# SuwoongHeo/neurecon

Measured on AMD Instinct MI355X. Metric: rays/sec (4096 rays x 128 samples, 8-layer x256 SDF MLP), higher is better.
Workload: dtype f16x3

## Files before the change

### neurecon_amd/csrc/nr_mlp.hip

```cpp
#include <algorithm>
#include <type_traits>
#include "nr_common.h"
#include "nr_mlp.h"
#include "nr_tgemm.h"

namespace nr {

using lds_ptr = __attribute__((address_space(3))) void*;

__device__ __forceinline__ void glds16(const char* gsrc, uint32_t lds_addr) {
  unsigned keep;
  asm volatile(
      "s_mov_b32 %0, m0\n\t"
      "s_mov_b32 m0, %2\n\t"
      "s_nop 0\n\t"
      "global_load_lds_dwordx4 %1, off\n\t"
      "s_mov_b32 m0, %0"
      : "=&s"(keep)
      : "v"(gsrc), "s"(lds_addr)
      : "memory");
}

__device__ __forceinline__ void glds16s(const char* sbase, uint32_t voff, uint32_t lds_addr) {
  unsigned keep;
// ... 398 lines not shown
    if (main) {
      if (e_cur) {
        const float4* eb = ws.slab_cur();
        const float4 e0 = eb[lane], e1 = eb[64 + lane];
        y0 = make_float4(act_bwd<P, ACTB>(y0.x, e0.x), act_bwd<P, ACTB>(y0.y, e0.y), act_bwd<P, ACTB>(y0.z, e0.z),
                         act_bwd<P, ACTB>(y0.w, e0.w));
        y1 = make_float4(act_bwd<P, ACTB>(y1.x, e1.x), act_bwd<P, ACTB>(y1.y, e1.y), act_bwd<P, ACTB>(y1.z, e1.z),
                         act_bwd<P, ACTB>(y1.w, e1.w));
      }
      if constexpr (NBO1 > 0) push2<NBO1>(Y, y0, y1);
    } else {
      emb(2 * c - NBO1, y0);
      emb(2 * c + 1 - NBO1, y1);
    }
    ws.flip();
  }
}

__device__ __noinline__ float embed_feature(int f, float x0, float x1, float x2, int nfreq) {
  if (f < 3) return f == 0 ? x0 : (f == 1 ? x1 : x2);
  const int fp = f - 3;
  if (fp >= 6 * nfreq) return 0.0f;
  const int band = fp / 6, m = fp - band * 6, c = m % 3;
  const float xc = c == 0 ? x0 : (c == 1 ? x1 : x2);
  const float v = fmul(xc, (float)(1 << band));
  return m < 3 ? sinf(v) : cosf(v);
}
__device__ __noinline__ void embed_backward(int f, float gf, float x0, float x1, float x2, int nfreq, float& n0,
                                            float& n1, float& n2) {
  float contrib;
  int c;
  if (f < 3) {
    contrib = gf;
    c = f;
  } else {
    const int fp = f - 3;
    if (fp >= 6 * nfreq) return;
    const int band = fp / 6, m = fp - band * 6;
    c = m % 3;
    const float freq = (float)(1 << band);
    const float xc = c == 0 ? x0 : (c == 1 ? x1 : x2);
    const float v = fmul(xc, freq);
    contrib = m < 3 ? fmul(fmul(gf, cosf(v)), freq) : fmul(fmul(gf, -sinf(v)), freq);
  }
  if (c == 0) n0 = fadd(n0, contrib);
  else if (c == 1) n1 = fadd(n1, contrib);
  else n2 = fadd(n2, contrib);
}

__device__ __forceinline__ float wave_sum4(float v) {
  v += __shfl_xor(v, 16);
  v += __shfl_xor(v, 32);
  return v;
}

struct SdfKArgs {
  const char* packed;
  SdfLayout L;
  const float* pts;
  int64_t P;
  float* sdf;
  float* nabla;
  float* feature;
  float4* scratch;
  int nfreq;
  const int* P_dev;
  int P_mult;
  float4* slabs;
  const int* tiles;
  const int* n_tiles;
  const char* f8_alt;
};

template <int P, bool NABLA>
__global__ __launch_bounds__(kThreads) void sdf_kernel(SdfKArgs a) {
  constexpr int CB = chunk_bytes(18);
  __shared__ __attribute__((aligned(16))) char smem[kRing * CB + (NABLA ? 2 * kSlabChunk : 0)];
  WStream<CB> ws{smem, NABLA ? smem + kRing * CB : nullptr, 0, 0, 0};
  const int lane = threadIdx.x & 63, wave = __builtin_amdgcn_readfirstlane(threadIdx.x >> 6);
  const int j = lane & 15, g = lane >> 4;
  const SdfLayout& L = a.L;
  const char* W = a.packed;
  auto OP = [&](int i) { return W + L.op_off[i]; };
  auto OPB = [&](int i) { return (int)L.op_bytes[i]; };
  const float* w8 = (const float*)(W + L.w8row0_off);
  const float b8 = *(const float*)(W + L.misc_off);
  float4* escr = uniform_ptr(a.scratch + (size_t)(blockIdx.x * kWaves + wave) * (8 * 16 * 64));
  const bool want_feat = a.feature != nullptr;

  ws.start(OP(F0), OPB(F0), OP(F0) + OPB(F0), OPB(F0));

  const int64_t Pn = a.P_dev ? min(a.P, (int64_t)(*a.P_dev) * a.P_mult) : a.P;
  for (int64_t base = (int64_t)blockIdx.x * kPointsPerWG; base < Pn; base += (int64_t)gridDim.x * kPointsPerWG) {
    const bool has_next = base + (int64_t)gridDim.x * kPointsPerWG < Pn;
    const int64_t p = base + wave * kTile + j;
    const bool valid = p < Pn;
    const int64_t pc = valid ? p : Pn - 1;
    const float x0 = a.pts[pc * 3 + 0], x1 = a.pts[pc * 3 + 1], x2 = a.pts[pc * 3 + 2];

    float4 E[4];
#pragma unroll
    for (int b = 0; b < 4; ++b) {
      const int f = 16 * b + 4 * g;
      E[b] = make_float4(embed_feature(f + 0, x0, x1, x2, a.nfreq), embed_feature(f + 1, x0, x1, x2, a.nfreq),
                         embed_feature(f + 2, x0, x1, x2, a.nfreq), embed_feature(f + 3, x0, x1, x2, a.nfreq));
    }
// ... 376 lines not shown
      wait_vmcnt(n);
    }
    __syncthreads();
    cur = nextr(cur);
  }
  __device__ __forceinline__ void flip_nowait() {
    __syncthreads();
    cur = nextr(cur);
  }
};

__device__ __forceinline__ f16x8 rd_frag(const float4* __restrict__ A, int i, int lane) {
  return as_h8(A[i * 64 + lane]);
}
template <int NS, class Stage>
__device__ __forceinline__ void mma4(const float4* __restrict__ A, const f16x8 (&bh)[kNC][12],
                                     const f16x8 (&bl)[kNC][12], f32x4 (&acc)[kNC][2], int lane, Stage&& stage) {
  f16x8 nh0 = rd_frag(A, 0, lane), nl0 = rd_frag(A, 1, lane);
  f16x8 nh1 = rd_frag(A, NS * 2, lane), nl1 = rd_frag(A, NS * 2 + 1, lane);
#pragma unroll
  for (int s = 0; s < NS; ++s) {
    const f16x8 h0 = nh0, l0 = nl0, h1 = nh1, l1 = nl1;
    if (s + 1 < NS) {
      nh0 = rd_frag(A, (s + 1) * 2, lane);
      nl0 = rd_frag(A, (s + 1) * 2 + 1, lane);
      nh1 = rd_frag(A, (NS + s + 1) * 2, lane);
      nl1 = rd_frag(A, (NS + s + 1) * 2 + 1, lane);
    }
    stage(s);
#pragma unroll
    for (int q = 0; q < kNC; ++q) {
      acc[q][0] = mfma16h(l0, bh[q][s], acc[q][0]);
      acc[q][1] = mfma16h(l1, bh[q][s], acc[q][1]);
      acc[q][0] = mfma16h(h0, bl[q][s], acc[q][0]);
      acc[q][1] = mfma16h(h1, bl[q][s], acc[q][1]);
      acc[q][0] = mfma16h(h0, bh[q][s], acc[q][0]);
      acc[q][1] = mfma16h(h1, bh[q][s], acc[q][1]);
    }
    if (s + 1 < NS) __builtin_amdgcn_sched_group_barrier(0x100, 4, 0);
    __builtin_amdgcn_sched_group_barrier(0x008, 6 * kNC, 0);
    __builtin_amdgcn_sched_barrier(0);
  }
}

struct Z4 {
  float4 z[kNC][2];
  float4 aux[2];
};

constexpr float kT = 144.26944f;
constexpr float kC = 0.0069314749f;

#ifdef NR_EXP_STAMPS
constexpr int kStampPh = 6;
__device__ unsigned long long g_nr_stamps[2048 * 8 * kStampPh];
__device__ __forceinline__ unsigned long long* stamp_lds() {
  __shared__ unsigned long long s_stamp[kW4 * kStampPh];
  return s_stamp;
}
__device__ __forceinline__ uint64_t stamp_now() { return __builtin_amdgcn_s_memtime(); }
__device__ __forceinline__ void stamp_add(int ph, uint64_t dt) {
  if ((threadIdx.x & 63) == 0) stamp_lds()[(threadIdx.x >> 6) * kStampPh + ph] += dt;
}
#define NR_STAMP(var) const uint64_t var = stamp_now()
#else
#define NR_STAMP(var)
#endif

enum { kSlot = 0, kLean = 1, kTab = 2 };
template <int KB, int NBO, int NXT_CB, bool AUX, bool TS, int MODE = kSlot, int NXT_MODE = kSlot, class WS,
          class Pre, class Epi>
__device__ __forceinline__ void op4(WS& ws, const char* __restrict__ op, const char* nxt, const f16x8 (&bh)[kNC][12],
                                    const f16x8 (&bl)[kNC][12], const float (&xinv)[kNC], Pend4& pd, Pre&& pre,
                                    Epi&& epi, int lane, float winv = 0.0f) {
  constexpr int CB = chunk_bytes(KB);
  constexpr bool LEAN = MODE == kLean;
  constexpr int FB = MODE != kSlot ? weight_bytes(KB) : CB;
  constexpr int NXT_FB = NXT_MODE != kSlot ? NXT_CB - 1024 : NXT_CB;
  static_assert(!LEAN || (!AUX && !TS), "lean ops carry no per-row data");
  constexpr int NCH = NBO / 2;
  static_assert(MODE != kTab || NCH * 512 <= kTabBytes, "bias table entries");
  constexpr int LA = WS::kRingN - 1;
  static_assert(NCH >= 2, "the 2-ahead stream needs >= 2 chunks per op");
  const int g = lane >> 4;
  Z4 zq{};
#pragma unroll
  for (int c = 0; c < NCH; ++c) {
    const char* opc = op;
    const char* nxc = nxt;
    asm volatile("" : "+s"(opc), "+s"(nxc));
    NR_STAMP(t0);
    int npend = 0;
    if (c + LA < NCH) {
      ws.template issue<FB>(opc + (c + LA) * CB);
      npend = WS::template npieces<FB>();
    } else if (nxc) {
      ws.template issue<NXT_FB>(nxc + (c + LA - NCH) * NXT_CB);
      npend = WS::template npieces<NXT_FB>();
      if constexpr (NXT_MODE == kTab) {
        if (c + LA == NCH) {
          ws.template dma_tab<NXT_CB>(nxc, ws.tcur ^ 1);
          npend += WS::ntab();
        }
      }
    }
    npend += pre(c);
    npend += pd.flush();
    NR_STAMP(t1);
    const float4* A = ws.buf();
    f32x4 acc[kNC][2] = {};
    mma4<KB / 2>(A, bh, bl, acc, lane, [&](int st) {
      if (c > 0) {
#pragma unroll
        for (int e = 0; e < 8; ++e)
          if (e * (KB / 2) / 8 == st) epi(c - 1, zq, e);
      }
    });
    NR_STAMP(t2);
    float wi;
// ... 190 lines not shown
};

template <int NMAIN, class WS>
struct BwdEpi4 {
  f16x8 (&oh)[kNC][12];
  f16x8 (&ol)[kNC][12];
  const float (&sc)[kNC];
  WS& ws;
  float4* park;
  int park_blk;
  float (&mrun)[kNC];
  Pend4& pd;
  int lane;
  int plane;
  float4 y[kNC][2];
  __device__ __forceinline__ void operator()(int c, const Z4& zz, int st) {
    if (2 * c < NMAIN) {
      const int q = st >> 2, k = st & 3;
      if (q >= kNC) return;
      if (k < 2) {
        const uint4 sw = *(const uint4*)((const char*)ws.slab_read() + ((kNC * k + q) * 64 + lane) * 16);
        y[q][k] = unpack24_mul(sw.x, sw.y, sw.z, zz.z[q][k]);
      } else if (k == 2) {
        mrun[q] = amax8(mrun[q], y[q][0], y[q][1]);
      } else {
        split8a(y[q][0], y[q][1], sc[q], oh[q][c], ol[q][c]);
        if (q == kNC - 1) ws.slab_consumed();
      }
    } else if (st == 7) {
#pragma unroll
      for (int q = 0; q < kNC; ++q) {
        pd.v[q] = zz.z[q][0];
        pd.v[kNC + q] = zz.z[q][1];
      }
      pend_chunk(pd, park, park_blk + 2 * c - NMAIN, plane, false);
    }
  }
};

struct NoPre4 {
  __device__ __forceinline__ int operator()(int) const { return 0; }
};

template <bool NABLA, bool FEAT, int STAGE_>
__global__ __attribute__((amdgpu_flat_work_group_size(STAGE_ == 3 ? 256 : kT4, STAGE_ == 3 ? 256 : kT4),
                          amdgpu_waves_per_eu(kWPE, kWPE)))
void sdf4_kernel(SdfKArgs a) {
  constexpr int STAGE = STAGE_ == 3 ? 0 : (STAGE_ == 4 ? 2 : STAGE_);
  constexpr bool COMPACT = STAGE_ == 4;
  constexpr int NW = STAGE_ == 3 ? 4 : kW4;
  static_assert(STAGE_ != 3 || (!NABLA && !FEAT), "narrow tiles: forward-only launches");
  static_assert(STAGE == 0 || (NABLA && !FEAT), "deferred nablas: no feature");
  constexpr int PPW = 16 * kNC * NW;
  constexpr int CB = chunk_bytes(18);
  constexpr int C16 = chunk_bytes(16), C4 = chunk_bytes(4), C14 = chunk_bytes(14), C18 = chunk_bytes(18);
  static_assert((size_t)kW4 * kNC * kSlabColBytes <= kScratchPerWG, "per-workgroup slab scratch");
  constexpr bool SLABS = NABLA && STAGE != 1;
  constexpr int RING = SLABS ? 3 : kFwdRing;
  constexpr bool TABF = !SLABS;
  constexpr int FM = TABF ? kTab : kSlot;
  constexpr int LDSB = RING * CB + (SLABS ? kSlabRing * kSlab4 : 0) + (TABF ? 2 * kTabBytes : 0);
  __shared__ __attribute__((aligned(16))) char smem[LDSB];
  static_assert(LDSB <= 160 * 1024, "LDS budget");
  static_assert(!TABF || RING * CB + 2 * kTabBytes == LDSB, "the bias table follows the weight ring");
  WStream4<CB, RING, NW> ws{smem, SLABS ? smem + RING * CB : nullptr, 0, 0, 0, 0, TABF ? smem + RING * CB : nullptr, 0};
  const int lane = threadIdx.x & 63, wave = __builtin_amdgcn_readfirstlane(threadIdx.x >> 6);
  const int j = lane & 15, g = lane >> 4;
  const char* W = a.packed;
  auto OP = [&](int i) {
    const char* w = W;
    asm volatile("" : "+s"(w));
    return w + sdf_op_off(i);
  };
  auto OPF8 = [&]() {
    const char* w = a.f8_alt;
    asm volatile("" : "+s"(w));
    return w ? w : OP(F8);
  };
  const float b8 = *(const float*)(W + a.L.misc_off);
  float4* escr = uniform_ptr((float4*)((char*)a.scratch + (size_t)(blockIdx.x * kW4 + wave) * (kNC * kSlabColBytes)));
  auto slab = [&](int l) {
    char* e = (char*)escr;
    asm volatile("" : "+s"(e));
    return (float4*)(e + l * kNC * kSlab24Layer);
  };

#ifdef NR_EXP_STAMPS
  if ((threadIdx.x & 63) == 0)
    for (int i = 0; i < kStampPh; ++i) stamp_lds()[wave * kStampPh + i] = 0;
#endif
  constexpr bool LEANR = STAGE == 2 || (NABLA && FEAT);
  constexpr int W16 = weight_bytes(16);
  if constexpr (STAGE == 2) ws.template start<W16, W16>(OP(B7), OP(B7) + C16);
  else if constexpr (TABF)
    ws.template start<weight_bytes(4), weight_bytes(4), weight_bytes(4), C4>(OP(F0), OP(F0) + C4, OP(F0) + 2 * C4, OP(F0));
  else ws.template start<C4, C4>(OP(F0), OP(F0) + C4);
  Pend4 pd{};
  NoPre4 nopre;
  const float kSpSlack = 0.0070f;

  const int64_t Pn = COMPACT      ? ((int64_t)(*a.n_tiles) + 15) / 16 * 16
                     : STAGE == 2 ? (int64_t)(*a.n_tiles) * kPointsPerWG / kW4
                                  : (a.P_dev ? min(a.P, (int64_t)(*a.P_dev) * a.P_mult) : a.P);
  for (int64_t base = (int64_t)blockIdx.x * PPW; base < Pn; base += (int64_t)gridDim.x * PPW) {
    const bool has_next = base + (int64_t)gridDim.x * PPW < Pn;
    int64_t p0 = base + wave * 16 * kNC;
    int plane = lane;
    uint32_t soff = 0;
    int64_t pl = 0;
    bool listed = true;
    if constexpr (COMPACT) {
      const int64_t n = *a.n_tiles;
      const int64_t w0 = p0 < n ? p0 : n - 16;
      const int e = a.tiles[w0 + j];
      const int e0 = __builtin_amdgcn_readfirstlane(a.tiles[w0]);
      listed = p0 < n && e >= 0;
      pl = e >= 0 ? e : e0;
      const uint32_t rt = (uint32_t)((pl >> 4) - (e0 >> 4)), js = (uint32_t)(pl & 15);
      plane = (int)(rt * (uint32_t)(kSlabColBytes / 16) + js + 16u * (uint32_t)g);
      soff = rt * (uint32_t)kSlabColBytes + (js + 16u * (uint32_t)g) * (uint32_t)kSlabVB;
      escr = uniform_ptr((float4*)((char*)a.slabs + (size_t)(e0 >> 4) * kSlabColBytes));
    } else if constexpr (STAGE == 2) {
      const int64_t ti = min(p0 / 16, (int64_t)(*a.n_tiles) - 1);
      const int64_t tile = a.tiles[ti];
      escr = uniform_ptr((float4*)((char*)a.slabs + (size_t)tile * kSlabColBytes));
      p0 = p0 / 16 < (int64_t)(*a.n_tiles) ? tile * 16 : a.P;
    } else if constexpr (STAGE == 1) {
      escr = uniform_ptr((float4*)((char*)a.slabs + (size_t)(p0 / 16) * kSlabColBytes));
    }
    const int64_t Pv = STAGE == 2 ? a.P : Pn;
    int64_t pq[kNC];
    bool valid[kNC];
    float xs[kNC][3];
#pragma unroll
    for (int q = 0; q < kNC; ++q) {
      const int64_t p = p0 + 16 * q + j;
      if constexpr (COMPACT) {
        valid[q] = listed;
        pq[q] = pl;
      } else {
        valid[q] = p < Pv;
        pq[q] = valid[q] ? p : Pv - 1;
      }
      xs[q][0] = a.pts[pq[q] * 3 + 0];
      xs[q][1] = a.pts[pq[q] * 3 + 1];
      xs[q][2] = a.pts[pq[q] * 3 + 2];
    }
    float4 E[kNC][4];
    float mE[kNC], xinv[kNC];
    f16x8 Uh[kNC][12], Ul[kNC][12], Vh[kNC][12], Vl[kNC][12];
    float mrun[kNC], m_in[kNC];
    auto next_scales = [&](int kb, float extra, const float (&floor_max)[kNC], float (&sc)[kNC]) {
      const float4 v = TABF ? ws.tab_entry(0)[8] : ws.buf()[2 * kb * 64 + 8];
#pragma unroll
      for (int q = 0; q < kNC; ++q) sc[q] = bound_scale(fmaxf(fmaf(v.y, m_in[q], v.z) + extra, floor_max[q]));
    };
    struct OpScal {
      float winv, R, B;
    };
    auto op_scal = [&](int opi) {
      const char* w = W;
      asm volatile("" : "+s"(w));
      typedef __attribute__((address_space(4))) const float cfloat;
      cfloat* rb = (cfloat*)(w + a.L.bound_off + 8 * opi);
      return OpScal{*(cfloat*)(w + a.L.winv_off + 4 * opi), rb[0], rb[1]};
    };
    auto finish = [&](const float (&sc)[kNC], float mscale = 1.0f) {
#pragma unroll
      for (int q = 0; q < kNC; ++q) {
        m_in[q] = max4_groups(mrun[q]) * mscale;
        mrun[q] = 0.0f;
        xinv[q] = 1.0f / sc[q];
      }
    };
    float zero2[kNC];
#pragma unroll
    for (int q = 0; q < kNC; ++q) zero2[q] = 0.0f;
    if constexpr (STAGE != 2) {
#pragma unroll
    for (int q = 0; q < kNC; ++q) {
#pragma unroll
      for (int b = 0; b < 4; ++b) {
        const int f = 16 * b + 4 * g;
        E[q][b] = make_float4(embed_feature(f + 0, xs[q][0], xs[q][1], xs[q][2], a.nfreq),
                              embed_feature(f + 1, xs[q][0], xs[q][1], xs[q][2], a.nfreq),
                              embed_feature(f + 2, xs[q][0], xs[q][1], xs[q][2], a.nfreq),
                              embed_feature(f + 3, xs[q][0], xs[q][1], xs[q][2], a.nfreq));
      }
      mE[q] = max4_groups(amax8(amax8(0.0f, E[q][0], E[q][1]), E[q][2], E[q][3]));
      const float sE = bound_scale(mE[q]);
      split8a(E[q][0], E[q][1], sE, Uh[q][0], Ul[q][0]);
      split8a(E[q][2], E[q][3], sE, Uh[q][1], Ul[q][1]);
      xinv[q] = 1.0f / sE;
    }
    float4* epark = slab(7);
    if constexpr (NABLA) {
      const uint32_t l = opaque_lane(lane);
#pragma unroll
      for (int q = 0; q < kNC; ++q)
#pragma unroll
        for (int b = 0; b < 4; ++b) {
          const uint32_t off = (((12 + b) * kNC + q) * 64 + l) * 16u;
          const f32x4 d = tof(E[q][b]);
          asm volatile("global_store_dwordx4 %0, %1, %2\n\ts_nop 1" : : "v"(off), "v"(d), "s"(epark) : "memory");
        }
    }
#pragma unroll
    for (int q = 0; q < kNC; ++q) {
      mrun[q] = 0.0f;
      m_in[q] = mE[q];
    }
    auto fwd_epi = [&](f16x8(&oh)[kNC][12], f16x8(&ol)[kNC][12], const float (&sc)[kNC], float4* sl) {
      return FwdEpi4<NABLA>{oh, ol, sc, sl, mrun, pd, lane};
    };

    {
      float sc[kNC];
      next_scales(4, kSpSlack, zero2, sc);
      op4<4, 16, C16, false, true, FM, FM>(ws, OP(F0), OP(F1), Uh, Ul, xinv, pd, nopre, fwd_epi(Vh, Vl, sc, slab(0)), lane);
      finish(sc, kC);
    }
    {
      float sc[kNC];
      next_scales(16, kSpSlack, zero2, sc);
      op4<16, 16, C16, false, true, FM, FM>(ws, OP(F1), OP(F2), Vh, Vl, xinv, pd, nopre, fwd_epi(Uh, Ul, sc, slab(1)), lane);
      finish(sc, kC);
    }
    {
      float sc[kNC];
      next_scales(16, kSpSlack, zero2, sc);
      op4<16, 16, C16, false, true, FM, FM>(ws, OP(F2), OP(F3), Uh, Ul, xinv, pd, nopre, fwd_epi(Vh, Vl, sc, slab(2)), lane);
      finish(sc, kC);
    }
    {
      float sc[kNC];
      next_scales(16, kSpSlack, mE, sc);
      op4<16, 14, C18, false, true, FM, FM>(ws, OP(F3), OP(F4), Vh, Vl, xinv, pd, nopre, fwd_epi(Uh, Ul, sc, slab(3)), lane);
      if constexpr (NABLA) {
        asm volatile("s_waitcnt vmcnt(0)" ::: "memory");
#pragma unroll
        for (int q = 0; q < kNC; ++q)
#pragma unroll
          for (int b = 0; b < 4; ++b) E[q][b] = fromf(*((const gf4*)epark + ((12 + b) * kNC + q) * 64 + lane));
      }
#pragma unroll
      for (int q = 0; q < kNC; ++q) {
        split8a(E[q][0], E[q][1], sc[q], Uh[q][7], Ul[q][7]);
        split8a(E[q][2], E[q][3], sc[q], Uh[q][8], Ul[q][8]);
        mrun[q] = fmaxf(mrun[q], mE[q] * (1.0f / kC));
      }
      finish(sc, kC);
    }
    {
      float sc[kNC];
      next_scales(18, kSpSlack, zero2, sc);
      op4<18, 16, C16, false, true, FM, FM>(ws, OP(F4), OP(F5), Uh, Ul, xinv, pd, nopre, fwd_epi(Vh, Vl, sc, slab(4)), lane);
      finish(sc, kC);
    }
    {
      float sc[kNC];
      next_scales(16, kSpSlack, zero2, sc);
      op4<16, 16, C16, false, true, FM, FM>(ws, OP(F5), OP(F6), Vh, Vl, xinv, pd, nopre, fwd_epi(Uh, Ul, sc, slab(5)), lane);
      finish(sc, kC);
    }
    {
      float sc[kNC];
      next_scales(16, kSpSlack, zero2, sc);
      op4<16, 16, C16, false, true, FM, FM>(ws, OP(F6), OP(F7), Uh, Ul, xinv, pd, nopre, fwd_epi(Vh, Vl, sc, slab(6)), lane);
      finish(sc, kC);
    }
    float sdf_part[kNC];
#pragma unroll
    for (int q = 0; q < kNC; ++q) sdf_part[q] = 0.0f;
    {
      float sc[kNC];
      next_scales(16, kSpSlack, zero2, sc);
      F7Epi4<NABLA, FEAT> epi{Uh, Ul, sc, slab(7), mrun, sdf_part, pd, lane};
      constexpr int NXT = ((NABLA && STAGE == 0) || FEAT) ? C16 : C4;
      const char* n;
      if constexpr (FEAT) n = OPF8();
      else n = (NABLA && STAGE == 0) ? OP(B7) : (has_next ? OP(F0) : nullptr);
      op4<16, 16, NXT, true, false, FM, FM>(ws, OP(F7), n, Vh, Vl, xinv, pd, nopre, epi, lane);
      finish(sc);
    }
#pragma unroll
    for (int q = 0; q < kNC; ++q) {
      const float sdf = wave_sum4(sdf_part[q]) + b8;
      if (valid[q] && g == 0) a.sdf[p0 + 16 * q + j] = sdf;
    }
    if constexpr (FEAT) {
      const int64_t pf = p0 < Pn ? p0 : Pn - 1;
      float4* fb = uniform_ptr((float4*)(a.feature + pf * 256));
      uint32_t frow[kNC];
#pragma unroll
      for (int q = 0; q < kNC; ++q) frow[q] = (uint32_t)(pq[q] - pf);
      auto epi = [&](int c, const Z4& zz, int st) {
        if (st != 7) return;
#pragma unroll
        for (int q = 0; q < kNC; ++q) {
          pd.v[2 * q] = zz.z[q][0];
          pd.v[2 * q + 1] = zz.z[q][1];
          const uint32_t r = opaque_lane(frow[q] * 64 + g);
          pd.o[2 * q] = r + (2 * c) * 4;
          pd.o[2 * q + 1] = r + (2 * c + 1) * 4;
        }
        pd.put(fb, 2 * kNC, kFeatNT);
      };
      constexpr int NXT = NABLA ? C16 : C4;
      const char* n = NABLA ? OP(B7) : (has_next ? OP(F0) : nullptr);
      op4<16, 16, NXT, false, false, FM, NABLA ? (LEANR ? kLean : kSlot) : FM>(ws, OPF8(), n, Uh, Ul, xinv, pd, nopre, epi,
                                                                               lane);
    }
    }
    if constexpr (NABLA && STAGE == 1) {
      pd.flush();
    }
    if constexpr (NABLA && STAGE != 1) {
      pd.flush();
      asm volatile("s_waitcnt vmcnt(0)" ::: "memory");
      OpScal osn{};
      if constexpr (LEANR) osn = op_scal(B7);
      float4* g7 = slab(7);
#pragma unroll
      for (int q = 0; q < kNC; ++q) {
        float4 G[16];
#pragma unroll
        for (int b = 0; b < 16; ++b) G[b] = fromf(*((const gf4*)g7 + (kNC * b + q) * 64 + (COMPACT ? plane : lane)));
        float m = 0.0f;
#pragma unroll
        for (int b = 0; b < 16; b += 2) m = amax8(m, G[b], G[b + 1]);
        m_in[q] = max4_groups(m);
        mrun[q] = 0.0f;
        const float sc = bound_scale(m_in[q]);
#pragma unroll
        for (int s = 0; s < 8; ++s) split8a(G[2 * s], G[2 * s + 1], sc, Uh[q][s], Ul[q][s]);
        xinv[q] = 1.0f / sc;
      }
      float4* park = slab(7);
      if constexpr (COMPACT) ws.stage_slab(slab(6), 0, soff);
      else ws.stage_slab(slab(6), 0);
      auto bwd = [&](auto kb_tag, auto nbo_tag, auto nmain_tag, auto nxt_tag, auto nxl_tag, int opi, const char* nxt,
                     f16x8(&ih)[kNC][12], f16x8(&il)[kNC][12], f16x8(&oh)[kNC][12], f16x8(&ol)[kNC][12], int lcur,
                     int park_blk, int lnext) {
        constexpr int KBo = decltype(kb_tag)::value, NBOo = decltype(nbo_tag)::value;
        constexpr int NMAIN = decltype(nmain_tag)::value, NXC = decltype(nxt_tag)::value;
        constexpr bool NXL = decltype(nxl_tag)::value;
        const OpScal os = osn;
        float sc[kNC];
        if constexpr (LEANR) {
          if (opi != B0) osn = op_scal(opi + 1);
#pragma unroll
          for (int q = 0; q < kNC; ++q) sc[q] = bound_scale(fmaxf(fmaf(os.R, m_in[q], os.B) + 0.0f, zero2[q]));
        } else {
          next_scales(KBo, 0.0f, zero2, sc);
        }
        auto pre = [&](int c) -> int {
          if constexpr (COMPACT) {
            if (2 * (c + 1) < NMAIN) return ws.stage_slab(slab(lcur), c + 1, soff);
            if (c + 1 == NBOo / 2 && lnext >= 0) return ws.stage_slab(slab(lnext), 0, soff);
          } else {
            if (2 * (c + 1) < NMAIN) return ws.stage_slab(slab(lcur), c + 1);
            if (c + 1 == NBOo / 2 && lnext >= 0) return ws.stage_slab(slab(lnext), 0);
          }
          return 0;
        };
        BwdEpi4<NMAIN, decltype(ws)> epi{oh, ol, sc, ws, park, park_blk, mrun, pd, lane, COMPACT ? plane : lane};
        constexpr int RM = LEANR ? kLean : kSlot, RMN = (LEANR && NXL) ? kLean : kSlot;
        op4<KBo, NBOo, NXC, false, false, RM, RMN>(ws, OP(opi), nxt, ih, il, xinv, pd, pre, epi, lane, os.winv);
        finish(sc);
      };
      using I0 = std::integral_constant<int, 0>;
      using I4 = std::integral_constant<int, 4>;
      using I14 = std::integral_constant<int, 14>;
      using I16 = std::integral_constant<int, 16>;
      using I18 = std::integral_constant<int, 18>;
      using IC16 = std::integral_constant<int, C16>;
      using IC14 = std::integral_constant<int, C14>;
      using IC4 = std::integral_constant<int, C4>;
      using LeanNext = std::true_type;
      using SlotNext = std::false_type;
      bwd(I16{}, I16{}, I16{}, IC16{}, LeanNext{}, B7, OP(B6), Uh, Ul, Vh, Vl, 6, 0, 5);
      bwd(I16{}, I16{}, I16{}, IC16{}, LeanNext{}, B6, OP(B5), Vh, Vl, Uh, Ul, 5, 0, 4);
      bwd(I16{}, I16{}, I16{}, IC16{}, LeanNext{}, B5, OP(B4), Uh, Ul, Vh, Vl, 4, 0, 3);
      bwd(I16{}, I18{}, I14{}, IC14{}, LeanNext{}, B4, OP(B3), Vh, Vl, Uh, Ul, 3, 0, 2);
      bwd(I14{}, I16{}, I16{}, IC16{}, LeanNext{}, B3, OP(B2), Uh, Ul, Vh, Vl, 2, 0, 1);
      bwd(I16{}, I16{}, I16{}, IC16{}, LeanNext{}, B2, OP(B1), Vh, Vl, Uh, Ul, 1, 0, 0);
      bwd(I16{}, I16{}, I16{}, IC16{}, LeanNext{}, B1, OP(B0), Uh, Ul, Vh, Vl, 0, 0, -1);
      if constexpr (STAGE == 2) bwd(I16{}, I4{}, I0{}, IC16{}, LeanNext{}, B0, has_next ? OP(B7) : nullptr, Vh, Vl, Uh, Ul, 0, 4, -1);
      else bwd(I16{}, I4{}, I0{}, IC4{}, SlotNext{}, B0, has_next ? OP(F0) : nullptr, Vh, Vl, Uh, Ul, 0, 4, -1);
      pd.flush();
      asm volatile("s_waitcnt vmcnt(0)" ::: "memory");
#pragma unroll
      for (int q = 0; q < kNC; ++q) {
        float n0 = 0.f, n1 = 0.f, n2 = 0.f;
#pragma unroll
        for (int b = 0; b < 4; ++b) {
          const float4 u = fromf(*((const gf4*)park + (kNC * b + q) * 64 + (COMPACT ? plane : lane)));
          const float4 v = fromf(*((const gf4*)park + (kNC * (4 + b) + q) * 64 + (COMPACT ? plane : lane)));
          const int f = 16 * b + 4 * g;
          embed_backward(f + 0, fadd(v.x, u.x), xs[q][0], xs[q][1], xs[q][2], a.nfreq, n0, n1, n2);
          embed_backward(f + 1, fadd(v.y, u.y), xs[q][0], xs[q][1], xs[q][2], a.nfreq, n0, n1, n2);
          embed_backward(f + 2, fadd(v.z, u.z), xs[q][0], xs[q][1], xs[q][2], a.nfreq, n0, n1, n2);
          embed_backward(f + 3, fadd(v.w, u.w), xs[q][0], xs[q][1], xs[q][2], a.nfreq, n0, n1, n2);
        }
        n0 = wave_sum4(n0);
        n1 = wave_sum4(n1);
        n2 = wave_sum4(n2);
        if (valid[q] && g == 0) {
          const int64_t p = COMPACT ? pq[q] : p0 + 16 * q + j;
          a.nabla[p * 3 + 0] = n0;
          a.nabla[p * 3 + 1] = n1;
          a.nabla[p * 3 + 2] = n2;
        }
      }
    }
  }
  pd.flush();
  wait_vmcnt(0);
#ifdef NR_EXP_STAMPS
  if ((threadIdx.x & 63) == 0 && blockIdx.x < 2048)
    for (int i = 0; i < kStampPh; ++i)
      g_nr_stamps[(blockIdx.x * kW4 + wave) * kStampPh + i] = stamp_lds()[wave * kStampPh + i];
#endif
}


template <int P, bool NABLA>
__global__ __launch_bounds__(kThreads) void siren_sdf_kernel(SdfKArgs a) {
  constexpr int CB = chunk_bytes(16);
  __shared__ __attribute__((aligned(16))) char smem[kRing * CB + (NABLA ? 2 * kSlabChunk : 0)];
  WStream<CB> ws{smem, NABLA ? smem + kRing * CB : nullptr, 0, 0, 0};
  const int lane = threadIdx.x & 63, wave = __builtin_amdgcn_readfirstlane(threadIdx.x >> 6);
  const int j = lane & 15, g = lane >> 4;
  const SdfLayout& L = a.L;
  const char* W = a.packed;
  auto OP = [&](int i) { return W + L.op_off[i]; };
  auto OPB = [&](int i) { return (int)L.op_bytes[i]; };
  const float* wl = (const float*)(W + L.w8row0_off);
  const float bl = *(const float*)(W + L.misc_off);
  float4* escr = uniform_ptr(a.scratch + (size_t)(blockIdx.x * kWaves + wave) * (8 * 16 * 64));
  const bool want_feat = a.feature != nullptr;

  ws.start(OP(S0), OPB(S0), OP(S0) + OPB(S0), OPB(S0));

  const int64_t Pn = a.P_dev ? min(a.P, (int64_t)(*a.P_dev) * a.P_mult) : a.P;
  for (int64_t base = (int64_t)blockIdx.x * kPointsPerWG; base < Pn; base += (int64_t)gridDim.x * kPointsPerWG) {
    const bool has_next = base + (int64_t)gridDim.x * kPointsPerWG < Pn;
    const int64_t p = base + wave * kTile + j;
    const bool valid = p < Pn;
    const int64_t pc = valid ? p : Pn - 1;
    const float x0 = a.pts[pc * 3 + 0], x1 = a.pts[pc * 3 + 1], x2 = a.pts[pc * 3 + 2];
    float4 E[4];
    E[0] = g == 0 ? make_float4(x0, x1, x2, 0.f) : make_float4(0.f, 0.f, 0.f, 0.f);
#pragma unroll
    for (int b = 1; b < 4; ++b) E[b] = make_float4(0.f, 0.f, 0.f, 0.f);
    float4 X[16], Y[16];
    float4* e_l[5];
#pragma unroll
    for (int l = 0; l < 5; ++l) e_l[l] = NABLA ? escr + l * 16 * 64 : nullptr;

    gemm_fwd<P, 0, 4, 16, ACT_SINE>(ws, OP(S0), OP(S1), OPB(S1), X, E, Y, e_l[0], nullptr, false, lane);
    gemm_fwd<P, 16, 0, 16, ACT_SINE>(ws, OP(S1), OP(S2), OPB(S2), Y, E, X, e_l[1], nullptr, false, lane);
    gemm_fwd<P, 16, 0, 16, ACT_SINE>(ws, OP(S2), OP(S3), OPB(S3), X, E, Y, e_l[2], nullptr, false, lane);
    gemm_fwd<P, 16, 0, 16, ACT_SINE>(ws, OP(S3), OP(S4), OPB(S4), Y, E, X, e_l[3], nullptr, false, lane);
    {
      const char* n = want_feat ? OP(SF) : (NABLA ? OP(SB4) : (has_next ? OP(S0) : nullptr));
      const int nb = want_feat ? OPB(SF) : (NABLA ? OPB(SB4) : OPB(S0));
      gemm_fwd<P, 16, 0, 16, ACT_SINE>(ws, OP(S4), n, nb, X, E, Y, e_l[4], nullptr, false, lane);
    }
    float part = 0.0f;
#pragma unroll
    for (int b = 0; b < 16; ++b) {
      const float4 w = *(const float4*)(wl + 16 * b + 4 * g);
      part = fmaf(Y[b].x, w.x, part);
      part = fmaf(Y[b].y, w.y, part);
// ... 1603 lines not shown
    PackBatch pb{};
    int64_t nmax = 0;
    for (int i = 0; i < nb; ++i) {
      const PackOp& op = ops[b0 + i];
      NR_REQUIRE(op.prec != NR_PREC_F16X3 || op.wmax, NR_ERR_ARG, "pack: f16x3 needs a max-|W| word");
      const int KB = op.in[0].nblk + op.in[1].nblk;
      const int NBO = op.out[0].nblk + op.out[1].nblk;
      pb.op[i] = op;
      pb.dst[i] = (uint32_t*)dst[b0 + i];
      pb.n[i] = (int64_t)(NBO / 2) * (2 * KB + 1) * 256;
      nmax = std::max(nmax, pb.n[i]);
    }
    int gmax = 1;
    for (int i = 0; i < nb; ++i)
      gmax = std::max(gmax, ((pb.op[i].out[0].nblk + pb.op[i].out[1].nblk) * 16 + kPackRowsPerWG - 1) / kPackRowsPerWG);
    NR_REQUIRE(gmax <= 32, NR_ERR_UNSUPPORTED, "pack: more than 512 output rows in one op");
    hipLaunchKernelGGL(pack_rows_kernel, dim3(gmax, nb), dim3(1024), 0, stream, pb);
    NR_HIP_CHECK(hipGetLastError());
    hipLaunchKernelGGL(pack_final_kernel, dim3(nb), dim3(256), 0, stream, pb);
    NR_HIP_CHECK(hipGetLastError());
    hipLaunchKernelGGL(pack_ops_kernel, dim3((unsigned)((nmax + 255) / 256), nb), dim3(256), 0, stream, pb);
    NR_HIP_CHECK(hipGetLastError());
  }
  return NR_OK;
}

int launch_pack_op(const PackOp& op, char* dst, hipStream_t stream) { return launch_pack_ops(&op, &dst, 1, stream); }

int launch_pack_vec(const float* src, int off, int nvalid, int n, char* dst, hipStream_t stream) {
  hipLaunchKernelGGL(pack_vec_kernel, dim3((n + 255) / 256), dim3(256), 0, stream, src, off, nvalid, n, (float*)dst);
  NR_HIP_CHECK(hipGetLastError());
  return NR_OK;
}

static int cu_count() {
  int dev = 0, cus = 256;
  if (hipGetDevice(&dev) == hipSuccess) (void)hipDeviceGetAttribute(&cus, hipDeviceAttributeMultiprocessorCount, dev);
  return cus;
}

static int grid_for(int64_t P, int ppw = kPointsPerWG) {
  const int cus = cu_count();
  const int64_t need = (P + ppw - 1) / ppw;
  return (int)(need < cus ? (need > 0 ? need : 1) : cus);
}

int launch_sdf(const SdfLayout& L, const void* packed, const float* pts, int64_t P, float* sdf, float* nabla,
               float* feature, int nfreq, void* ws, size_t ws_bytes, hipStream_t stream, const int* P_dev,
               int P_mult, const void* f8_alt) {
  if (P <= 0) return NR_OK;
  const int grid = grid_for(P);
  NR_REQUIRE(!f8_alt || (feature && L.prec == NR_PREC_F16X3 && !L.siren), NR_ERR_ARG,
             "sdf: an op in F8's place needs the f16x3 softplus net and a feature buffer");
  SdfKArgs a{(const char*)packed, L, pts, P, sdf, nabla, feature, (float4*)ws, nfreq, P_dev, P_mult, nullptr, nullptr,
             nullptr, (const char*)f8_alt};
  ProfScope prof(nabla ? (feature ? "sdf_nabla_feat" : "sdf_nabla") : (feature ? "sdf_feat" : "sdf_fwd"), (double)P,
                 stream, P_dev, P_mult);
  if (L.siren) {
    if (nabla) {
      const size_t need = (size_t)grid * kScratchPerWG;
      NR_REQUIRE(ws && ws_bytes >= need, NR_ERR_WORKSPACE, "sdf nabla workspace too small");
      if (L.prec == NR_PREC_F16X3)
        hipLaunchKernelGGL((siren_sdf_kernel<NR_PREC_F16X3, true>), dim3(grid), dim3(kThreads), 0, stream, a);
      else hipLaunchKernelGGL((siren_sdf_kernel<NR_PREC_FP32, true>), dim3(grid), dim3(kThreads), 0, stream, a);
    } else {
      if (L.prec == NR_PREC_F16X3)
        hipLaunchKernelGGL((siren_sdf_kernel<NR_PREC_F16X3, false>), dim3(grid), dim3(kThreads), 0, stream, a);
      else hipLaunchKernelGGL((siren_sdf_kernel<NR_PREC_FP32, false>), dim3(grid), dim3(kThreads), 0, stream, a);
    }
    NR_HIP_CHECK(hipGetLastError());
    return NR_OK;
  }
  if (nabla) {
    const size_t need = (size_t)grid * kScratchPerWG;
    NR_REQUIRE(ws && ws_bytes >= need, NR_ERR_WORKSPACE, "sdf nabla workspace too small");
    if (L.prec == NR_PREC_F16X3) {
      if (feature) hipLaunchKernelGGL((sdf4_kernel<true, true, 0>), dim3(grid), dim3(kT4), 0, stream, a);
      else hipLaunchKernelGGL((sdf4_kernel<true, false, 0>), dim3(grid), dim3(kT4), 0, stream, a);
    }
    else hipLaunchKernelGGL((sdf_kernel<NR_PREC_FP32, true>), dim3(grid), dim3(kThreads), 0, stream, a);
  } else {
    if (L.prec == NR_PREC_F16X3) {
      if (feature) hipLaunchKernelGGL((sdf4_kernel<false, true, 0>), dim3(grid), dim3(kT4), 0, stream, a);
      else if (P <= (int64_t)64 * cu_count())
        hipLaunchKernelGGL((sdf4_kernel<false, false, 3>), dim3(grid_for(P, 64)), dim3(256), 0, stream, a);
      else hipLaunchKernelGGL((sdf4_kernel<false, false, 0>), dim3(grid), dim3(kT4), 0, stream, a);
    }
    else hipLaunchKernelGGL((sdf_kernel<NR_PREC_FP32, false>), dim3(grid), dim3(kThreads), 0, stream, a);
  }
  NR_HIP_CHECK(hipGetLastError());
  return NR_OK;
}

int launch_sdf_deferred(const SdfLayout& L, const void* packed, const float* pts, int64_t P, float* sdf, float* nabla,
                        int nfreq, float4* slabs, const int* tiles, const int* n_tiles, int stage, hipStream_t stream) {
  if (P <= 0) return NR_OK;
  NR_REQUIRE(L.prec == NR_PREC_F16X3 && !L.siren, NR_ERR_UNSUPPORTED, "deferred nablas: f16x3 softplus nets");
  SdfKArgs a{(const char*)packed, L, pts, P, sdf, nabla, nullptr, nullptr, nfreq, nullptr, 0, slabs, tiles, n_tiles};
  if (stage == 1) {
    ProfScope prof("sdf_nabla_fwd", (double)P, stream);
    hipLaunchKernelGGL((sdf4_kernel<true, false, 1>), dim3(grid_for(P)), dim3(kT4), 0, stream, a);
  } else if (stage == 2) {
    ProfScope prof("sdf_nabla_bwd", (double)P, stream, n_tiles, 16);
    hipLaunchKernelGGL((sdf4_kernel<true, false, 2>), dim3(grid_for(P)), dim3(kT4), 0, stream, a);
  } else {
    NR_REQUIRE(stage == 4, NR_ERR_ARG, "deferred nablas: bad stage");
    ProfScope prof("sdf_nabla_bwd", (double)P, stream, n_tiles, 1);
    hipLaunchKernelGGL((sdf4_kernel<true, false, 4>), dim3(grid_for(P)), dim3(kT4), 0, stream, a);
  }
  NR_HIP_CHECK(hipGetLastError());
  return NR_OK;
}

int launch_nerf(const NerfLayout& L, const void* packed, const float* x4, const float* vdir, int64_t vdiv,
                int64_t vmod, int64_t P, float* sigma, float* rgb, hipStream_t stream, const int* P_dev) {
  if (P <= 0) return NR_OK;
  const int grid = grid_for(P);
  NerfKArgs a{(const char*)packed, L, x4, vdir, vdiv, vmod, P, sigma, rgb, P_dev};
  ProfScope prof("nerf", (double)P, stream, P_dev, 1);
  if (L.prec == NR_PREC_F16X3) hipLaunchKernelGGL(nerf4_kernel, dim3(grid), dim3(kT4), 0, stream, a);
  else hipLaunchKernelGGL((nerf_kernel<NR_PREC_FP32>), dim3(grid), dim3(kThreads), 0, stream, a);
  NR_HIP_CHECK(hipGetLastError());
  return NR_OK;
}

int launch_nerf_train32_fwd(const NerfLayout& L, const void* packed, const float* xe, const float* ve, int64_t P,
                            float* const* h, float* feat, float* hv, float* sigma, float* rgb, hipStream_t stream) {
  if (P <= 0) return NR_OK;
  NR_REQUIRE(L.prec == NR_PREC_FP32, NR_ERR_ARG, "nerf train forward: needs the fp32 render pack");
  NerfTrainFwdArgs a{};
  a.packed = (const char*)packed;
  a.L = L;
  a.xe = xe;
  a.ve = ve;
  a.P = P;
  for (int i = 0; i < 8; ++i) a.h[i] = h[i];
  a.feat = feat;
  a.hv = hv;
  a.sigma = sigma;
  a.rgb = rgb;
  ProfScope prof("nerf_train32_fwd", (double)P, stream);
  hipLaunchKernelGGL(nerf_train32_fwd_kernel, dim3(grid_for(P)), dim3(kThreads), 0, stream, a);
  NR_HIP_CHECK(hipGetLastError());
  return NR_OK;
}

int launch_nerf_train32_bwd(const NerfBwdLayout& B, const void* packed, const float* rgb, const float* hv,
                            const float* const* h, const float* g_rgb, const float* g_sigma, int64_t P, float* g3,
                            float* ghv, float* g_feat, float* const* gz, hipStream_t stream,
                            bool f16x3) {
// ... 33 lines not shown
  return NR_OK;
}

int launch_radiance(const RadLayout& L, const void* packed, const float* x, const float* vdir, int64_t vdiv,
                    int64_t vmod, const float* normals, const float* feature, int64_t P, float* rgb, int nfreq_view,
                    hipStream_t stream, const int* P_dev, const void* r0_fold) {
  if (P <= 0) return NR_OK;
  const int grid = grid_for(P);
  NR_REQUIRE(!r0_fold || (L.prec == NR_PREC_F16X3 && !L.siren && L.D == 4), NR_ERR_ARG,
             "radiance: the folded layer 0 needs the f16x3 ReLU D=4 net");
  RadKArgs a{(const char*)packed, L, x, vdir, vdiv, vmod, normals, feature, P, rgb, nfreq_view, P_dev,
             (const char*)r0_fold};
  ProfScope prof("radiance", (double)P, stream, P_dev, 1);
  const bool h3 = L.prec == NR_PREC_F16X3;
#define NR_RAD_LAUNCH(KBS, ACT, D)                                                                            \
  do {                                                                                                        \
    if (h3) hipLaunchKernelGGL((radiance_kernel<NR_PREC_F16X3, KBS, ACT, D>), dim3(grid), dim3(kThreads), 0, \
                               stream, a);                                                                    \
    else hipLaunchKernelGGL((radiance_kernel<NR_PREC_FP32, KBS, ACT, D>), dim3(grid), dim3(kThreads), 0,     \
                            stream, a);                                                                       \
  } while (0)
  if (L.kbs != 2 && L.kbs != 4) {
    set_error("radiance: unsupported small-input block count");
    return NR_ERR_UNSUPPORTED;
  }
  if (h3 && !L.siren && L.D == 4) {
    if (r0_fold) {
      if (L.kbs == 2) hipLaunchKernelGGL((rad4_kernel<2, true>), dim3(grid), dim3(kT4), 0, stream, a);
      else hipLaunchKernelGGL((rad4_kernel<4, true>), dim3(grid), dim3(kT4), 0, stream, a);
    } else if (L.kbs == 2) hipLaunchKernelGGL((rad4_kernel<2, false>), dim3(grid), dim3(kT4), 0, stream, a);
    else hipLaunchKernelGGL((rad4_kernel<4, false>), dim3(grid), dim3(kT4), 0, stream, a);
  } else if (!L.siren && L.D == 4) {
    if (L.kbs == 2) NR_RAD_LAUNCH(2, ACT_RELU, 4); else NR_RAD_LAUNCH(4, ACT_RELU, 4);
  } else if (!L.siren && L.D == 5) {
    if (L.kbs == 2) NR_RAD_LAUNCH(2, ACT_RELU, 5); else NR_RAD_LAUNCH(4, ACT_RELU, 5);
  } else if (L.D == 4) {
    if (L.kbs == 2) NR_RAD_LAUNCH(2, ACT_SINE, 4); else NR_RAD_LAUNCH(4, ACT_SINE, 4);
  } else {
    if (L.kbs == 2) NR_RAD_LAUNCH(2, ACT_SINE, 5); else NR_RAD_LAUNCH(4, ACT_SINE, 5);
  }
#undef NR_RAD_LAUNCH
  NR_HIP_CHECK(hipGetLastError());
  return NR_OK;
}

}

#ifdef NR_EXP_STAMPS
extern "C" int nr_exp_stamps(unsigned long long* out, int n) {
  return hipMemcpyFromSymbol(out, HIP_SYMBOL(nr::g_nr_stamps), sizeof(unsigned long long) * (size_t)n) == hipSuccess
             ? nr::kW4 * nr::kStampPh
             : -1;
}
#endif
```

Measured before the change: 711,900.

## Share positional-encoding sin/cos across lanes via bpermute in nabla kernels

Replaces the per-feature positional encoding, which calls sinf/cosf once for every embedded feature in each lane, with a scheme where each 16-lane group evaluates five sincos pairs. Values are then routed to the lanes that need them with ds_bpermute, in both the forward embedding and the analytic-gradient backward pass. The path applies only to nabla kernels (stages 0 with feature, 2 and 4). It adds a hard requirement that nfreq equals 6, plus extra timing-stamp instrumentation that is compiled only under a debug flag. The aim is to cut redundant transcendental evaluation, paid for with extra cross-lane permutes and select instructions.

```diff
diff --git a/neurecon_amd/csrc/nr_mlp.hip b/neurecon_amd/csrc/nr_mlp.hip
--- a/neurecon_amd/csrc/nr_mlp.hip
+++ b/neurecon_amd/csrc/nr_mlp.hip
@@ -474,6 +474,89 @@
   v += __shfl_xor(v, 16);
   v += __shfl_xor(v, 32);
   return v;
+}
+
+constexpr int kEncSlots = 5, kEncBands = 6;
+struct Enc4 {
+  float s[kEncSlots], c[kEncSlots];
+};
+__device__ __noinline__ float2 embed_sincos(float v) { return make_float2(sinf(v), cosf(v)); }
+__device__ __forceinline__ void enc_eval(Enc4& t, const float (&x)[3], int g) {
+  float x0 = x[0], x1 = x[1], x2 = x[2];
+  asm volatile("" : "+v"(x0), "+v"(x1), "+v"(x2));
+#pragma unroll
+  for (int s = 0; s < kEncSlots; ++s) {
+    const uint32_t a = (uint32_t)g + 4u * s, band = (a * 11u) >> 5 , c = a - 3u * band;
+    float xc = c == 1u ? x1 : x0;
+    xc = c == 2u ? x2 : xc;
+    const float2 r = embed_sincos(fmul(xc, __uint_as_float(0x3f800000u + (band << 23))));
+    t.s[s] = r.x;
+    t.c[s] = r.y;
+  }
+}
+constexpr uint32_t enc_src(int f, bool deriv) {
+  const int fp = f - 3;
+  if (fp < 0 || fp >= 6 * kEncBands) return 0xffu;
+  const int band = fp / 6, m = fp % 6, a = band * 3 + m % 3;
+  return (uint32_t)((a & 3) | ((a >> 2) << 2) | (((m >= 3) != deriv) ? 32 : 0));
+}
+constexpr uint32_t enc_meta(int f) {
+  if (f < 3) return (uint32_t)(f | 64);
+  const int fp = f - 3;
+  if (fp >= 6 * kEncBands) return 0xffu;
+  const int band = fp / 6, m = fp % 6;
+  return (uint32_t)((m % 3) | (band << 2) | (m >= 3 ? 32 : 0));
+}
+template <int F0, bool DERIV>
+__device__ __forceinline__ float enc_pull(const Enc4& t, int g, int j) {
+  constexpr uint32_t c0 = enc_src(F0, DERIV), c1 = enc_src(F0 + 4, DERIV), c2 = enc_src(F0 + 8, DERIV),
+                     c3 = enc_src(F0 + 12, DERIV);
+  constexpr uint32_t word = c0 | (c1 << 8) | (c2 << 16) | (c3 << 24);
+  const uint32_t code = (word >> (8 * g)) & 0xffu;
+  const int addr = (int)((((code & 3u) << 4) | (uint32_t)j) << 2);
+  float out = 0.0f;
+#pragma unroll
+  for (uint32_t id = 0; id < 16; ++id) {
+    if ((c0 >> 2) != id && (c1 >> 2) != id && (c2 >> 2) != id && (c3 >> 2) != id) continue;
+    const float src = (id & 8) ? t.c[id & 7] : t.s[id & 7];
+    const float v = __int_as_float(__builtin_amdgcn_ds_bpermute(addr, __float_as_int(src)));
+    out = (code >> 2) == id ? v : out;
+  }
+  return out;
+}
+template <int B>
+__device__ __forceinline__ float4 enc_rows(const Enc4& t, const float (&x)[3], int g, int j) {
+  if constexpr (16 * B + 3 >= 3 + 6 * kEncBands + 12) {
+    float z = 0.0f;
+    asm volatile("" : "+v"(z));
+    return make_float4(z, z, z, z);
+  }
+  float v[4];
+  v[0] = enc_pull<16 * B + 0, false>(t, g, j);
+  v[1] = enc_pull<16 * B + 1, false>(t, g, j);
+  v[2] = enc_pull<16 * B + 2, false>(t, g, j);
+  v[3] = enc_pull<16 * B + 3, false>(t, g, j);
+  if constexpr (B == 0) {
+#pragma unroll
+    for (int r = 0; r < 3; ++r) v[r] = g == 0 ? x[r] : v[r];
+  }
+  return make_float4(v[0], v[1], v[2], v[3]);
+}
+template <int F0>
+__device__ __forceinline__ void enc_row_bwd(const Enc4& t, float gf, int g, int j, float& n0, float& n1,
+                                            float& n2) {
+  constexpr uint32_t m0 = enc_meta(F0), m1 = enc_meta(F0 + 4), m2 = enc_meta(F0 + 8), m3 = enc_meta(F0 + 12);
+  if constexpr (m0 == 0xffu && m1 == 0xffu && m2 == 0xffu && m3 == 0xffu) return;
+  constexpr uint32_t word = m0 | (m1 << 8) | (m2 << 16) | (m3 << 24);
+  const uint32_t meta = (word >> (8 * g)) & 0xffu;
+  const float tv = __uint_as_float(__float_as_uint(enc_pull<F0, true>(t, g, j)) ^ ((meta & 32u) << 26));
+  const float freq = __uint_as_float(0x3f800000u + (((meta >> 2) & 7u) << 23));
+  const float contrib = (meta & 64u) ? gf : fmul(fmul(gf, tv), freq);
+  const uint32_t c = meta & 3u;
+  const float s0 = fadd(n0, contrib), s1 = fadd(n1, contrib), s2 = fadd(n2, contrib);
+  n0 = c == 0u ? s0 : n0;
+  n1 = c == 1u ? s1 : n1;
+  n2 = c == 2u ? s2 : n2;
 }
 
 struct SdfKArgs {
@@ -956,8 +1039,9 @@
 constexpr float kC = 0.0069314749f;
 
 #ifdef NR_EXP_STAMPS
-constexpr int kStampPh = 6;
-__device__ unsigned long long g_nr_stamps[2048 * 8 * kStampPh];
+constexpr int kStampPh = 9;
+constexpr int kStampSlot = 2048 * 8 * kStampPh;
+__device__ unsigned long long g_nr_stamps[6 * kStampSlot];
 __device__ __forceinline__ unsigned long long* stamp_lds() {
   __shared__ unsigned long long s_stamp[kW4 * kStampPh];
   return s_stamp;
@@ -967,8 +1051,14 @@
   if ((threadIdx.x & 63) == 0) stamp_lds()[(threadIdx.x >> 6) * kStampPh + ph] += dt;
 }
 #define NR_STAMP(var) const uint64_t var = stamp_now()
+#define NR_STAMP_VAR(var) uint64_t var = 0
+#define NR_STAMP_SET(var) var = stamp_now()
+#define NR_STAMP_ADD(ph, dt) stamp_add(ph, dt)
 #else
 #define NR_STAMP(var)
+#define NR_STAMP_VAR(var)
+#define NR_STAMP_SET(var)
+#define NR_STAMP_ADD(ph, dt)
 #endif
 
 enum { kSlot = 0, kLean = 1, kTab = 2 };
@@ -1265,6 +1355,11 @@
   static_assert(STAGE_ != 3 || (!NABLA && !FEAT), "narrow tiles: forward-only launches");
   static_assert(STAGE == 0 || (NABLA && !FEAT), "deferred nablas: no feature");
   constexpr int PPW = 16 * kNC * NW;
+#ifdef NR_EXP_ROW_ENC
+  constexpr bool ENC4 = false;
+#else
+  constexpr bool ENC4 = NABLA && STAGE != 1 && !(!FEAT && STAGE_ == 0);
+#endif
   constexpr int CB = chunk_bytes(18);
   constexpr int C16 = chunk_bytes(16), C4 = chunk_bytes(4), C14 = chunk_bytes(14), C18 = chunk_bytes(18);
   static_assert((size_t)kW4 * kNC * kSlabColBytes <= kScratchPerWG, "per-workgroup slab scratch");
@@ -1317,6 +1412,10 @@
                                   : (a.P_dev ? min(a.P, (int64_t)(*a.P_dev) * a.P_mult) : a.P);
   for (int64_t base = (int64_t)blockIdx.x * PPW; base < Pn; base += (int64_t)gridDim.x * PPW) {
     const bool has_next = base + (int64_t)gridDim.x * PPW < Pn;
+    NR_STAMP_VAR(ts0);
+    NR_STAMP_VAR(ts1);
+    NR_STAMP_VAR(te0);
+    NR_STAMP_SET(ts0);
     int64_t p0 = base + wave * 16 * kNC;
     int plane = lane;
     uint32_t soff = 0;
@@ -1392,13 +1491,23 @@
     if constexpr (STAGE != 2) {
 #pragma unroll
     for (int q = 0; q < kNC; ++q) {
-#pragma unroll
-      for (int b = 0; b < 4; ++b) {
-        const int f = 16 * b + 4 * g;
-        E[q][b] = make_float4(embed_feature(f + 0, xs[q][0], xs[q][1], xs[q][2], a.nfreq),
-                              embed_feature(f + 1, xs[q][0], xs[q][1], xs[q][2], a.nfreq),
-                              embed_feature(f + 2, xs[q][0], xs[q][1], xs[q][2], a.nfreq),
-                              embed_feature(f + 3, xs[q][0], xs[q][1], xs[q][2], a.nfreq));
+      if constexpr (ENC4) {
+        const int ge = (int)opaque_lane(g), je = (int)opaque_lane(j);
+        Enc4 t;
+        enc_eval(t, xs[q], ge);
+        E[q][0] = enc_rows<0>(t, xs[q], ge, je);
+        E[q][1] = enc_rows<1>(t, xs[q], ge, je);
+        E[q][2] = enc_rows<2>(t, xs[q], ge, je);
+        E[q][3] = enc_rows<3>(t, xs[q], ge, je);
+      } else {
+#pragma unroll
+        for (int b = 0; b < 4; ++b) {
+          const int f = 16 * b + 4 * g;
+          E[q][b] = make_float4(embed_feature(f + 0, xs[q][0], xs[q][1], xs[q][2], a.nfreq),
+                                embed_feature(f + 1, xs[q][0], xs[q][1], xs[q][2], a.nfreq),
+                                embed_feature(f + 2, xs[q][0], xs[q][1], xs[q][2], a.nfreq),
+                                embed_feature(f + 3, xs[q][0], xs[q][1], xs[q][2], a.nfreq));
+        }
       }
       mE[q] = max4_groups(amax8(amax8(0.0f, E[q][0], E[q][1]), E[q][2], E[q][3]));
       const float sE = bound_scale(mE[q]);
@@ -1427,6 +1536,7 @@
       return FwdEpi4<NABLA>{oh, ol, sc, sl, mrun, pd, lane};
     };
 
+    NR_STAMP_SET(ts1);
     {
       float sc[kNC];
       next_scales(4, kSpSlack, zero2, sc);
@@ -1496,6 +1606,7 @@
       op4<16, 16, NXT, true, false, FM, FM>(ws, OP(F7), n, Vh, Vl, xinv, pd, nopre, epi, lane);
       finish(sc);
     }
+    NR_STAMP_SET(te0);
 #pragma unroll
     for (int q = 0; q < kNC; ++q) {
       const float sdf = wave_sum4(sdf_part[q]) + b8;
@@ -1523,6 +1634,7 @@
       const char* n = NABLA ? OP(B7) : (has_next ? OP(F0) : nullptr);
       op4<16, 16, NXT, false, false, FM, NABLA ? (LEANR ? kLean : kSlot) : FM>(ws, OPF8(), n, Uh, Ul, xinv, pd, nopre, epi,
                                                                                lane);
+      NR_STAMP_SET(te0);
     }
     }
     if constexpr (NABLA && STAGE == 1) {
@@ -1592,6 +1704,9 @@
       using IC4 = std::integral_constant<int, C4>;
       using LeanNext = std::true_type;
       using SlotNext = std::false_type;
+      if constexpr (STAGE == 2) {
+        NR_STAMP_SET(ts1);
+      }
       bwd(I16{}, I16{}, I16{}, IC16{}, LeanNext{}, B7, OP(B6), Uh, Ul, Vh, Vl, 6, 0, 5);
       bwd(I16{}, I16{}, I16{}, IC16{}, LeanNext{}, B6, OP(B5), Vh, Vl, Uh, Ul, 5, 0, 4);
       bwd(I16{}, I16{}, I16{}, IC16{}, LeanNext{}, B5, OP(B4), Uh, Ul, Vh, Vl, 4, 0, 3);
@@ -1601,20 +1716,44 @@
       bwd(I16{}, I16{}, I16{}, IC16{}, LeanNext{}, B1, OP(B0), Uh, Ul, Vh, Vl, 0, 0, -1);
       if constexpr (STAGE == 2) bwd(I16{}, I4{}, I0{}, IC16{}, LeanNext{}, B0, has_next ? OP(B7) : nullptr, Vh, Vl, Uh, Ul, 0, 4, -1);
       else bwd(I16{}, I4{}, I0{}, IC4{}, SlotNext{}, B0, has_next ? OP(F0) : nullptr, Vh, Vl, Uh, Ul, 0, 4, -1);
+      NR_STAMP_SET(te0);
       pd.flush();
       asm volatile("s_waitcnt vmcnt(0)" ::: "memory");
 #pragma unroll
       for (int q = 0; q < kNC; ++q) {
         float n0 = 0.f, n1 = 0.f, n2 = 0.f;
-#pragma unroll
-        for (int b = 0; b < 4; ++b) {
+        auto grad = [&](int b) {
           const float4 u = fromf(*((const gf4*)park + (kNC * b + q) * 64 + (COMPACT ? plane : lane)));
           const float4 v = fromf(*((const gf4*)park + (kNC * (4 + b) + q) * 64 + (COMPACT ? plane : lane)));
-          const int f = 16 * b + 4 * g;
-          embed_backward(f + 0, fadd(v.x, u.x), xs[q][0], xs[q][1], xs[q][2], a.nfreq, n0, n1, n2);
-          embed_backward(f + 1, fadd(v.y, u.y), xs[q][0], xs[q][1], xs[q][2], a.nfreq, n0, n1, n2);
-          embed_backward(f + 2, fadd(v.z, u.z), xs[q][0], xs[q][1], xs[q][2], a.nfreq, n0, n1, n2);
-          embed_backward(f + 3, fadd(v.w, u.w), xs[q][0], xs[q][1], xs[q][2], a.nfreq, n0, n1, n2);
+          return make_float4(fadd(v.x, u.x), fadd(v.y, u.y), fadd(v.z, u.z), fadd(v.w, u.w));
+        };
+        if constexpr (ENC4) {
+          const int ge = (int)opaque_lane(g), je = (int)opaque_lane(j);
+          Enc4 t;
+          enc_eval(t, xs[q], ge);
+          const float4 g0 = grad(0), g1 = grad(1), g2 = grad(2);
+          enc_row_bwd<0>(t, g0.x, ge, je, n0, n1, n2);
+          enc_row_bwd<1>(t, g0.y, ge, je, n0, n1, n2);
+          enc_row_bwd<2>(t, g0.z, ge, je, n0, n1, n2);
+          enc_row_bwd<3>(t, g0.w, ge, je, n0, n1, n2);
+          enc_row_bwd<16>(t, g1.x, ge, je, n0, n1, n2);
+          enc_row_bwd<17>(t, g1.y, ge, je, n0, n1, n2);
+          enc_row_bwd<18>(t, g1.z, ge, je, n0, n1, n2);
+          enc_row_bwd<19>(t, g1.w, ge, je, n0, n1, n2);
+          enc_row_bwd<32>(t, g2.x, ge, je, n0, n1, n2);
+          enc_row_bwd<33>(t, g2.y, ge, je, n0, n1, n2);
+          enc_row_bwd<34>(t, g2.z, ge, je, n0, n1, n2);
+          enc_row_bwd<35>(t, g2.w, ge, je, n0, n1, n2);
+        } else {
+#pragma unroll
+          for (int b = 0; b < 4; ++b) {
+            const float4 gr = grad(b);
+            const int f = 16 * b + 4 * g;
+            embed_backward(f + 0, gr.x, xs[q][0], xs[q][1], xs[q][2], a.nfreq, n0, n1, n2);
+            embed_backward(f + 1, gr.y, xs[q][0], xs[q][1], xs[q][2], a.nfreq, n0, n1, n2);
+            embed_backward(f + 2, gr.z, xs[q][0], xs[q][1], xs[q][2], a.nfreq, n0, n1, n2);
+            embed_backward(f + 3, gr.w, xs[q][0], xs[q][1], xs[q][2], a.nfreq, n0, n1, n2);
+          }
         }
         n0 = wave_sum4(n0);
         n1 = wave_sum4(n1);
@@ -1627,13 +1766,20 @@
         }
       }
     }
+    NR_STAMP(te1);
+    NR_STAMP_ADD(6, ts1 - ts0);
+    NR_STAMP_ADD(7, te1 - te0);
+    NR_STAMP_ADD(8, te1 - ts0);
   }
   pd.flush();
   wait_vmcnt(0);
 #ifdef NR_EXP_STAMPS
   if ((threadIdx.x & 63) == 0 && blockIdx.x < 2048)
-    for (int i = 0; i < kStampPh; ++i)
-      g_nr_stamps[(blockIdx.x * kW4 + wave) * kStampPh + i] = stamp_lds()[wave * kStampPh + i];
+    for (int i = 0; i < kStampPh; ++i) {
+      const unsigned long long v = stamp_lds()[wave * kStampPh + i];
+      g_nr_stamps[(blockIdx.x * kW4 + wave) * kStampPh + i] = v;
+      g_nr_stamps[(1 + STAGE_) * kStampSlot + (blockIdx.x * kW4 + wave) * kStampPh + i] = v;
+    }
 #endif
 }
 
@@ -3343,6 +3489,8 @@
   const int grid = grid_for(P);
   NR_REQUIRE(!f8_alt || (feature && L.prec == NR_PREC_F16X3 && !L.siren), NR_ERR_ARG,
              "sdf: an op in F8's place needs the f16x3 softplus net and a feature buffer");
+  NR_REQUIRE(L.siren || L.prec != NR_PREC_F16X3 || nfreq == kEncBands, NR_ERR_UNSUPPORTED,
+             "sdf: the f16x3 softplus net encodes 6 bands");
   SdfKArgs a{(const char*)packed, L, pts, P, sdf, nabla, feature, (float4*)ws, nfreq, P_dev, P_mult, nullptr, nullptr,
              nullptr, (const char*)f8_alt};
   ProfScope prof(nabla ? (feature ? "sdf_nabla_feat" : "sdf_nabla") : (feature ? "sdf_feat" : "sdf_fwd"), (double)P,
@@ -3387,6 +3535,7 @@
                         int nfreq, float4* slabs, const int* tiles, const int* n_tiles, int stage, hipStream_t stream) {
   if (P <= 0) return NR_OK;
   NR_REQUIRE(L.prec == NR_PREC_F16X3 && !L.siren, NR_ERR_UNSUPPORTED, "deferred nablas: f16x3 softplus nets");
+  NR_REQUIRE(nfreq == kEncBands, NR_ERR_UNSUPPORTED, "sdf: the f16x3 softplus net encodes 6 bands");
   SdfKArgs a{(const char*)packed, L, pts, P, sdf, nabla, nullptr, nullptr, nfreq, nullptr, 0, slabs, tiles, n_tiles};
   if (stage == 1) {
     ProfScope prof("sdf_nabla_fwd", (double)P, stream);
@@ -3526,4 +3675,11 @@
              ? nr::kW4 * nr::kStampPh
              : -1;
 }
+extern "C" int nr_exp_stamps_stage(int stage, unsigned long long* out, int n) {
+  if (stage < 0 || stage > 4 || n > nr::kStampSlot) return -1;
+  return hipMemcpyFromSymbol(out, HIP_SYMBOL(nr::g_nr_stamps), sizeof(unsigned long long) * (size_t)n,
+                             sizeof(unsigned long long) * (size_t)(1 + stage) * nr::kStampSlot) == hipSuccess
+             ? nr::kW4 * nr::kStampPh
+             : -1;
+}
 #endif
```

New measurement: 724,600 (median of 6 runs). +1.8%, better.
